# lisqzqng/Video-based-gait-analysis-for-dementia

Hardware: AMD Instinct MI355X
Metric: frames/sec (224x224, seq=16) (higher is better)
Workload: dtype f32

## Files before the change

video-based-gait-analysis-for-dementia_amd/csrc/conv_stem.hip:

```cpp
#include "kernels.h"

namespace grk {

typedef float f32x4 __attribute__((ext_vector_type(4)));

namespace {

__global__ __launch_bounds__(256) void conv_stem_f32(const ConvArgs a) {
    const int lane = threadIdx.x & 63, l15 = lane & 15, lq = lane >> 4;
    const int row = blockIdx.x * 4 + (threadIdx.x >> 6);
    if (row >= a.N * a.Ho) return;
    const int n = row / a.Ho, y = row - n * a.Ho;
    const float* w = a.w;
    float bw[7][4];
#pragma unroll
    for (int s = 0; s < 7; ++s)
#pragma unroll
        for (int nt = 0; nt < 4; ++nt) bw[s][nt] = w[(s * 4 + nt) * 64 + lane];
    float bias[4];
#pragma unroll
    for (int nt = 0; nt < 4; ++nt) bias[nt] = a.bias[nt * 16 + l15];
    const float* rowp[7];
    int kxm1[7];
    bool yok[7];
    const float* inb = a.in + ((size_t)n * a.in_ctot + a.in_coff) * a.H * a.W;
#pragma unroll
    for (int s = 0; s < 7; ++s) {
        const int k = 4 * s + lq, kk = k < 27 ? k : 26, c = kk / 9, t = kk - 9 * c, ky = t / 3, kx = t - 3 * ky;
        const int yin = 2 * y + ky - 1;
        yok[s] = yin >= 0 && yin < a.H;
        rowp[s] = inb + ((size_t)c * a.H + (yok[s] ? yin : 0)) * a.W;
        kxm1[s] = kx - 1;
    }
    auto fetch = [&](int x0, float (&v)[7]) {
#pragma unroll
        for (int s = 0; s < 7; ++s) {
            const int xi = 2 * (x0 + l15) + kxm1[s];
            const bool ok = yok[s] && xi >= 0 && xi < a.W;
            const float t = rowp[s][ok ? xi : 0];
            v[s] = ok ? t : 0.f;
        }
    };
    float cur[7], nxt[7];
    fetch(0, cur);
    float* ob = a.out + (((size_t)n * a.out_ctot + a.out_coff + l15) * a.Ho + y) * a.Wo + 4 * lq;
    const size_t cstride = (size_t)16 * a.Ho * a.Wo;
    for (int x0 = 0; x0 < a.Wo; x0 += 16) {
        fetch(x0 + 16 < a.Wo ? x0 + 16 : x0, nxt);
        f32x4 acc[4];
#pragma unroll
        for (int nt = 0; nt < 4; ++nt) acc[nt] = f32x4{0.f, 0.f, 0.f, 0.f};
#pragma unroll
        for (int s = 0; s < 7; ++s)
#pragma unroll
            for (int nt = 0; nt < 4; ++nt) acc[nt] = __builtin_amdgcn_mfma_f32_16x16x4f32(cur[s], bw[s][nt], acc[nt], 0, 0, 0);
#pragma unroll
        for (int nt = 0; nt < 4; ++nt) {
            f32x4 v = acc[nt] + bias[nt];
            if (a.relu) {
#pragma unroll
                for (int r = 0; r < 4; ++r) v[r] = fmaxf(v[r], 0.f);
            }
            *reinterpret_cast<f32x4*>(ob + nt * cstride + x0) = v;
        }
#pragma unroll
        for (int s = 0; s < 7; ++s) cur[s] = nxt[s];
    }
}

}

bool conv_stem_eligible(int cin, int cout, int ks, int stride, int h, int w, int n_add) {
    return cin == 3 && cout == 64 && ks == 3 && stride == 2 && n_add == 0 && h % 2 == 0 && w % 32 == 0;
}

void pack_stem_weights(const double* w_folded , float* out ) {
    for (int s = 0; s < 7; ++s)
        for (int nt = 0; nt < 4; ++nt)
            for (int lq = 0; lq < 4; ++lq)
                for (int l15 = 0; l15 < 16; ++l15) {
                    const int k = 4 * s + lq, co = 16 * nt + l15;
                    out[(s * 4 + nt) * 64 + lq * 16 + l15] = k < 27 ? (float)w_folded[(size_t)co * 27 + k] : 0.f;
                }
}

hipError_t launch_conv_stem(ConvArgs a, hipStream_t s) {
    if (!conv_stem_eligible(a.Cin, a.Cout, a.ks, a.stride, a.H, a.W, a.n_add) || a.Ho * 2 != a.H || a.Wo * 2 != a.W) return hipErrorInvalidValue;
    const int rows = a.N * a.Ho;
    return launch_k(conv_stem_f32, dim3((rows + 3) / 4), dim3(256), 0, s, a);
}

}
```

video-based-gait-analysis-for-dementia_amd/csrc/grnet.cpp:

```cpp
#include "../../include/grnet_hip.h"

#include <hip/hip_runtime.h>

#include <cmath>
#include <cstdio>
#include <cstdlib>
#include <algorithm>
#include <cstring>
#include <map>
#include <memory>
#include <string>
#include <tuple>
#include <unordered_map>
#include <vector>

#include "kernels.h"

using namespace grk;

namespace grk { thread_local GraphRecorder* g_recorder = nullptr; }

namespace {

constexpr double kBnEps = 1e-5;
// ... 2040 lines not shown
        GraphKey key{n, frames, o};
        auto it = graphs.find(key);
        constexpr size_t kMaxGraphs = 16;
        if (it == graphs.end()) {
            bool seen = false;
            for (const GraphKey& k : seen_once) seen |= !(k < key) && !(key < k);
            if (!seen) {
                if (seen_once.size() >= 64) seen_once.erase(seen_once.begin());
                seen_once.push_back(key);
                return enqueue(frames, n, o, s);
            }
            if (graphs.size() >= kMaxGraphs) {
                auto lru = graphs.begin();
                for (auto g = graphs.begin(); g != graphs.end(); ++g)
                    if (g->second.last_use < lru->second.last_use) lru = g;
                (void)hipGraphExecDestroy(lru->second.exec);
                graphs.erase(lru);
            }
        }
        if (it == graphs.end()) {
            hipGraph_t g = nullptr;
            HIP_TRY(hipGraphCreate(&g, 0));
            GraphRecorder recorder;
            recorder.graph = g;
            static const int edges_env = GRNET_AB(GRAPH_EDGES, 0);
            recorder.edge_order = edges_env;
            g_recorder = &recorder;
            int rc = enqueue(frames, n, o, s);
            g_recorder = nullptr;
            if (rc) { hipGraphDestroy(g); return rc; }
            hipError_t e = hipSuccess;
            if (recorder.edge_order) {
                auto add = [&](std::vector<hipGraphNode_t>& from, std::vector<hipGraphNode_t>& to) {
                    if (e == hipSuccess && !from.empty()) e = hipGraphAddDependencies(g, from.data(), to.data(), from.size());
                };
                if (recorder.edge_order == 2) { add(recorder.cross_from, recorder.cross_to); add(recorder.chain_from, recorder.chain_to); }
                else { add(recorder.chain_from, recorder.chain_to); add(recorder.cross_from, recorder.cross_to); }
                if (e != hipSuccess) { hipGraphDestroy(g); return fail(GRNET_EHIP, std::string("hipGraphAddDependencies: ") + hipGetErrorString(e)); }
            }
            hipGraphExec_t ge = nullptr;
            e = hipGraphInstantiate(&ge, g, nullptr, nullptr, 0);
            hipGraphDestroy(g);
            if (e != hipSuccess) return fail(GRNET_EHIP, std::string("hipGraphInstantiate: ") + hipGetErrorString(e));
            it = graphs.emplace(key, GraphEntry{ge, 0}).first;
        }
        it->second.last_use = ++graph_clock;
        HIP_TRY(hipGraphLaunch(it->second.exec, s));
        return 0;
    }
};

extern "C" {

const char* grnet_version(void) { return "grnet_hip 0.1 (gfx950, fp32 MFMA)"; }

int grnet_create(grnet_t** out_handle, int device_id, int dtype, int max_frames) {
    if (!out_handle || max_frames < 1 || max_frames > 2048 || (dtype != 0 && dtype != 1)) return GRNET_EINVAL;
    *out_handle = nullptr;
    int ndev = 0;
    if (hipGetDeviceCount(&ndev) != hipSuccess || device_id < 0 || device_id >= ndev) return GRNET_EHIP;
    DeviceGuard guard(device_id);
    std::unique_ptr<grnet> h(new grnet());
    h->device = device_id;
    h->max_frames = max_frames;
    h->dtype = dtype;
    if (const char* ml = getenv("GRNET_MULTI_LANE")) h->multi_lane = atoi(ml) != 0;
    if (const char* wn = getenv("GRNET_WINO")) h->wino_mode = atoi(wn) != 0;
    h->build_plan();
    int rc = h->allocate();
    if (rc) { fprintf(stderr, "grnet_create: %s\n", h->err.c_str()); return rc; }
    if (conv_init() != hipSuccess || conv_bf16_init() != hipSuccess || conv_bf16_chain_init() != hipSuccess || conv_bf16_roll_init() != hipSuccess) { fprintf(stderr, "grnet_create: conv_init failed\n"); return GRNET_EHIP; }
    *out_handle = h.release();
    return 0;
}

int grnet_load_tensor(grnet_t* h, const char* key, const void* host_ptr, const int64_t* shape, int ndim, int dtype) {
    if (!h || !key || (!host_ptr && ndim >= 0 && dtype == GRNET_DTYPE_F32) || ndim < 0 || ndim > 8) return GRNET_EINVAL;
    if (h->finalized) return h->fail(GRNET_ESTATE, "grnet_load_tensor after grnet_finalize_weights");
    if (dtype == GRNET_DTYPE_I64) return 0;
    if (dtype != GRNET_DTYPE_F32) return h->fail(GRNET_EINVAL, std::string("unsupported dtype for ") + key);
    HostTensor t;
    size_t numel = 1;
    for (int i = 0; i < ndim; ++i) { t.shape.push_back(shape[i]); numel *= (size_t)shape[i]; }
    t.data.assign(static_cast<const float*>(host_ptr), static_cast<const float*>(host_ptr) + numel);
    h->tensors[key] = std::move(t);
    return 0;
}

int grnet_load_smpl(grnet_t* h, const float* v_template, const float* shapedirs, const float* posedirs, const float* J_regressor,
                    const float* lbs_weights, const int32_t* parents, const float* J_regressor_extra) {
    if (!h || !v_template || !shapedirs || !posedirs || !J_regressor || !lbs_weights || !parents || !J_regressor_extra)
        return GRNET_EINVAL;
    DeviceGuard guard(h->device);
    const int V = 6890;
    for (int i = 0; i < 24; ++i)
        if (parents[i] >= i || (i > 0 && parents[i] < 0)) return h->fail(GRNET_EINVAL, "SMPL parents must be topologically ordered");
    auto up = [&](const float* src, size_t n, const float** dst) {
        std::vector<float> tmp(src, src + n);
        float* p = nullptr;
        int rc = h->upload(tmp, &p);
        *dst = p;
        return rc;
    };
    int rc;
    {
        const size_t C = (size_t)V * 3;
        std::vector<float> blend((size_t)kBlendK * C, 0.f);
// ... 680 lines not shown
```

video-based-gait-analysis-for-dementia_amd/csrc/head_kernels.hip:

```cpp
#include "kernels.h"

namespace grk {

#define GRK_TRY(expr) do { hipError_t _e = (expr); if (_e != hipSuccess) return _e; } while (0)

typedef float f32x4 __attribute__((ext_vector_type(4)));
typedef float f32x2 __attribute__((ext_vector_type(2)));

__device__ __forceinline__ float wave_sum(float v) {
#pragma unroll
    for (int o = 32; o > 0; o >>= 1) v += __shfl_xor(v, o, 64);
    return v;
}
__device__ __forceinline__ float wave_max(float v) {
#pragma unroll
    for (int o = 32; o > 0; o >>= 1) v = fmaxf(v, __shfl_xor(v, o, 64));
    return v;
}

__global__ __launch_bounds__(256) void fuse_sum_kernel(const SumArgs a) {
    const int HW = a.H * a.W, n = blockIdx.x / a.C, c = blockIdx.x - n * a.C;
    const float inv_w = 1.0f / (float)a.W;
    for (int pix = threadIdx.x * 4; pix < HW; pix += 1024) {
        f32x4 v = f32x4{0.f, 0.f, 0.f, 0.f};
// ... 174 lines not shown
    double m[6];
#pragma unroll
    for (int k = 0; k < 6; ++k) m[k] = maps[(size_t)n * mstride + k];
    const int iw = mstride >= 10 ? (int)maps[(size_t)n * mstride + 6] : 0, ih = mstride >= 10 ? (int)maps[(size_t)n * mstride + 7] : 0;
    const double t2[6] = {1.0, 0.0, iw > 0 ? maps[(size_t)n * mstride + 8] : 0.0, 0.0, 1.0, iw > 0 ? maps[(size_t)n * mstride + 9] : 0.0};
    const float mean[3] = {0.485f, 0.456f, 0.406f}, stdv[3] = {0.229f, 0.224f, 0.225f};
    for (int i = blockIdx.x * 256 + threadIdx.x; i < 224 * 224; i += gridDim.x * 256) {
        const int y = i / 224, x = i - y * 224;
        int val[3];
        if (iw <= 0) {
            cv_warp_px(src, H, W, m, x, y, val);
        } else {
            const int X0 = cv_round((t2[1] * y + t2[2]) * 1024.0) + 16, Y0 = cv_round((t2[4] * y + t2[5]) * 1024.0) + 16;
            const int X = (X0 + cv_round(t2[0] * x * 1024.0)) >> 5, Y = (Y0 + cv_round(t2[3] * x * 1024.0)) >> 5;
            const int sx = min(max(X >> 5, -32768), 32767), sy = min(max(Y >> 5, -32768), 32767);
            const int ax = X & 31, ay = Y & 31;
            const int wt[4] = {(32 - ax) * (32 - ay), ax * (32 - ay), (32 - ax) * ay, ax * ay};
            int sum[3] = {0, 0, 0};
#pragma unroll
            for (int t = 0; t < 4; ++t) {
                const int ix = sx + (t & 1), iy = sy + (t >> 1);
                if (wt[t] != 0 && ix >= 0 && ix < iw && iy >= 0 && iy < ih) {
                    int v[3];
                    cv_warp_px(src, H, W, m, ix, iy, v);
                    sum[0] += v[0] * wt[t]; sum[1] += v[1] * wt[t]; sum[2] += v[2] * wt[t];
                }
            }
#pragma unroll
            for (int c = 0; c < 3; ++c) val[c] = (sum[c] * 32 + 16384) >> 15;
        }
#pragma unroll
        for (int c = 0; c < 3; ++c) out[((size_t)n * 3 + c) * (224 * 224) + i] = ((float)val[bgr ? 2 - c : c] / 255.f - mean[c]) / stdv[c];
    }
}

hipError_t launch_crop_normalise_cv(const unsigned char* img, int H, int W, int per_image, const double* maps, int mstride, int bgr, float* out, int N,
                                    hipStream_t s) {
    if (mstride != 6 && mstride != 10) return hipErrorInvalidValue;
    GRK_TRY(launch_k(crop_normalise_cv_kernel, dim3(49, N), dim3(256), 0, s, img, H, W, per_image, maps, mstride, bgr, out));
    return hipSuccess;
}

hipError_t launch_crop_normalise(const unsigned char* img, int H, int W, int per_image, const float* bbox, float scale, int bgr,
                                 float* out, int N, hipStream_t s) {
    GRK_TRY(launch_k(crop_normalise_kernel, dim3(49, N), dim3(256), 0, s, img, H, W, per_image, bbox, scale, bgr, out));
    return hipSuccess;
}

constexpr int kPoolChunk = 448, kPoolStride = kPoolChunk + 4;
__global__ __launch_bounds__(384) void attn_pool_kernel(const float* __restrict__ heat, int heat_ctot, float* __restrict__ stats,
                                                          const float* __restrict__ featA, int CA, const float* __restrict__ featB,
                                                          int CB, float* __restrict__ part, int P) {
    __shared__ __align__(16) float prob[32 * kPoolStride];
    const int n = blockIdx.x, tid = threadIdx.x, lane = tid & 63, l15 = lane & 15, lq = lane >> 4;
    const int pbeg = blockIdx.z * kPoolChunk;
    for (int u = tid; u < 32 * (kPoolChunk / 4); u += 384) {
        const int j = u / (kPoolChunk / 4), q = u - j * (kPoolChunk / 4);
        f32x4 v = {0.f, 0.f, 0.f, 0.f};
        if (j < 24) v = *reinterpret_cast<const f32x4*>(heat + ((size_t)n * heat_ctot + 1 + j) * P + pbeg + 4 * q);
        *reinterpret_cast<f32x4*>(prob + j * kPoolStride + 4 * q) = v;
    }
    __syncthreads();
    for (int j = (tid >> 6) * 4; j < (tid >> 6) * 4 + 4; ++j) {
        float* row = prob + j * kPoolStride;
        float hv[kPoolChunk / 64], m = -INFINITY;
#pragma unroll
        for (int i = 0; i < kPoolChunk / 64; ++i) { hv[i] = row[lane + 64 * i]; m = fmaxf(m, hv[i]); }
        m = wave_max(m);
        float sum = 0.f;
#pragma unroll
        for (int i = 0; i < kPoolChunk / 64; ++i) { const float e = expf(hv[i] - m); row[lane + 64 * i] = e; sum += e; }
        sum = wave_sum(sum);
        if (lane == 0 && blockIdx.y == 0) {
            float* st = stats + (((size_t)n * kPoolSplit + blockIdx.z) * 24 + j) * 2;
            st[0] = m;
            st[1] = sum;
        }
    }
    const int ct = blockIdx.y * 6 + (tid >> 6);
    const int c = ct * 16 + l15;
    const float* frow = (c < CA ? featA + ((size_t)n * CA + c) * P : featB + ((size_t)n * CB + (c - CA)) * P) + pbeg + 4 * lq;
    f32x4 fa[4];
#pragma unroll
    for (int g = 0; g < 4; ++g) fa[g] = *reinterpret_cast<const f32x4*>(frow + 16 * g);
    __syncthreads();
    const float* b0 = prob + l15 * kPoolStride + 4 * lq;
    const float* b1 = prob + (16 + l15) * kPoolStride + 4 * lq;
    f32x4 acc0 = {0.f, 0.f, 0.f, 0.f}, acc1 = {0.f, 0.f, 0.f, 0.f};
    for (int p0 = 0; p0 < kPoolChunk; p0 += 64) {
        const int pn = p0 + 64 < kPoolChunk ? p0 + 64 : p0;
#pragma unroll
        for (int g = 0; g < 4; ++g) {
            const f32x4 f = fa[g];
            fa[g] = *reinterpret_cast<const f32x4*>(frow + pn + 16 * g);
            const f32x4 u = *reinterpret_cast<const f32x4*>(b0 + p0 + 16 * g), v = *reinterpret_cast<const f32x4*>(b1 + p0 + 16 * g);
#pragma unroll
            for (int k = 0; k < 4; ++k) {
                acc0 = __builtin_amdgcn_mfma_f32_16x16x4f32(f[k], u[k], acc0, 0, 0, 0);
                acc1 = __builtin_amdgcn_mfma_f32_16x16x4f32(f[k], v[k], acc1, 0, 0, 0);
            }
        }
    }
    float* o = part + (((size_t)n * kPoolSplit + blockIdx.z) * (CA + CB) + ct * 16 + 4 * lq) * 24;
#pragma unroll
    for (int r = 0; r < 4; ++r) {
        o[r * 24 + l15] = acc0[r];
        if (l15 < 8) o[r * 24 + 16 + l15] = acc1[r];
    }
}

size_t softmax_pool_ws_floats(int N) { return (size_t)N * kPoolStatsFloats + (size_t)N * kPoolSplit * 192 * 24; }

hipError_t launch_softmax_pool(const float* heat, int heat_ctot, const float* featA, int CA, const float* featB, int CB,
                               float* outA, float* outB, float* stats_ws, int N, int P, hipStream_t s) {
    (void)outA; (void)outB;
    if (CA != 128 || CB != 64 || P != kPoolChunk * kPoolSplit) return hipErrorInvalidValue;
    float* part = stats_ws + (size_t)N * kPoolStatsFloats;
    GRK_TRY(launch_k(attn_pool_kernel, dim3(N, (CA + CB) / 96, kPoolSplit), dim3(384), 0, s, heat, heat_ctot, stats_ws, featA, CA, featB,
                       CB, part, P));
    return hipGetLastError();
}

__device__ __forceinline__ void rot6d_to_rotmat_dev(const float* x, float* R) {
    const float a1x = x[0], a1y = x[2], a1z = x[4], a2x = x[1], a2y = x[3], a2z = x[5];
    const float n1 = fmaxf(sqrtf(a1x * a1x + a1y * a1y + a1z * a1z), 1e-6f);
    const float b1x = a1x / n1, b1y = a1y / n1, b1z = a1z / n1;
    const float d = b1x * a2x + b1y * a2y + b1z * a2z;
    const float ux = a2x - d * b1x, uy = a2y - d * b1y, uz = a2z - d * b1z;
    const float n2 = fmaxf(sqrtf(ux * ux + uy * uy + uz * uz), 1e-6f);
    const float b2x = ux / n2, b2y = uy / n2, b2z = uz / n2;
    const float b3x = b1y * b2z - b1z * b2y, b3y = b1z * b2x - b1x * b2z, b3z = b1x * b2y - b1y * b2x;
    R[0] = b1x; R[1] = b2x; R[2] = b3x;
    R[3] = b1y; R[4] = b2y; R[5] = b3y;
    R[6] = b1z; R[7] = b2z; R[8] = b3z;
}

__device__ __forceinline__ void rotmat_to_aa_dev(const float* R, float* aa) {
    const float m00 = R[0], m01 = R[3], m02 = R[6];
    const float m10 = R[1], m11 = R[4], m12 = R[7];
    const float m20 = R[2], m21 = R[5], m22 = R[8];
    float q0, q1, q2, q3, t;
    if (m22 < 1e-6f) {
        if (m00 > m11) { t = 1.f + m00 - m11 - m22; q0 = m12 - m21; q1 = t; q2 = m01 + m10; q3 = m20 + m02; }
        else           { t = 1.f - m00 + m11 - m22; q0 = m20 - m02; q1 = m01 + m10; q2 = t; q3 = m12 + m21; }
    } else {
        if (m00 < -m11) { t = 1.f - m00 - m11 + m22; q0 = m01 - m10; q1 = m20 + m02; q2 = m12 + m21; q3 = t; }
        else            { t = 1.f + m00 + m11 + m22; q0 = t; q1 = m12 - m21; q2 = m20 - m02; q3 = m01 - m10; }
    }
    const float sc = 0.5f / sqrtf(t);
    q0 *= sc; q1 *= sc; q2 *= sc; q3 *= sc;
    const float s2 = q1 * q1 + q2 * q2 + q3 * q3;
    const float sn = sqrtf(s2);
    const float two_theta = 2.f * (q0 < 0.f ? atan2f(-sn, -q0) : atan2f(sn, q0));
    const float k = s2 > 0.f ? two_theta / sn : 2.f;
    float a0 = q1 * k, a1 = q2 * k, a2 = q3 * k;
    aa[0] = isnan(a0) ? 0.f : a0;
    aa[1] = isnan(a1) ? 0.f : a1;
    aa[2] = isnan(a2) ? 0.f : a2;
}

template <bool FROM_PARTS>
__global__ __launch_bounds__(256) void head_tail_kernel(const float* __restrict__ part, const float* __restrict__ zstats, float* __restrict__ plf, float* __restrict__ csf, TailWeights w,
                                                          float* __restrict__ rot6d, float* __restrict__ shape,
                                                          float* __restrict__ cam, float* __restrict__ rotmat,
                                                          float* __restrict__ theta) {
    __shared__ float s_plf[128 * 24];
    __shared__ __align__(16) float s_csf[64 * 24];
    __shared__ float s_pose[24 * 6];
    __shared__ float s_sc[13];
    __shared__ float s_pp[4][144];
// ... 351 lines not shown
```

video-based-gait-analysis-for-dementia_amd/csrc/hr_fuse.hip:

```cpp
#include "kernels.h"

namespace grk {

typedef float f32x4 __attribute__((ext_vector_type(4)));
typedef float f32x2 __attribute__((ext_vector_type(2)));

namespace {

template <int LW> struct VecOf;
template <> struct VecOf<1> { typedef float type; };
template <> struct VecOf<2> { typedef f32x2 type; };
template <> struct VecOf<4> { typedef f32x4 type; };
__device__ __forceinline__ float comp(float v, int) { return v; }
__device__ __forceinline__ float comp(f32x2 v, int r) { return v[r]; }
__device__ __forceinline__ float comp(f32x4 v, int r) { return v[r]; }

template <int NB, int I>
struct OutGeom {
    static constexpr int CI = 32 << I, WI = 56 >> I, BR = 8 >> I, NSRC = NB - 1 - I, NT = CI / 16;
    static constexpr int NSPLIT = NT < 4 ? NT : 4, KS = 4 / NSPLIT, NPW = NT / NSPLIT;
    static constexpr int VW = WI % 4 == 0 ? 4 : 2, WV = WI / VW, NV = CI * BR * WV;
};
template <int NB, int I, int S>
struct SrcGeom {
// ... 29 lines not shown
    }
#pragma unroll
    for (int g = 0; g < Q::KSW / 4; ++g)
#pragma unroll
        for (int u = 0; u < G::NPW; ++u)
            R.b[g][u] = *reinterpret_cast<const f32x4*>(src.w + ((size_t)((ksel * (Q::KSW / 4) + g) * G::NT + nsel * G::NPW + u) * 64 + lane) * 4);
}

template <int NB, int I, int S>
__device__ __forceinline__ void src_compute(const SrcRegs<NB, I, S>& R, float* T, int lane, int nsel, int ksel) {
    typedef SrcGeom<NB, I, S> Q;
    typedef OutGeom<NB, I> G;
    const int l15 = lane & 15, lq = lane >> 4;
    f32x4 acc[Q::MT][G::NPW];
#pragma unroll
    for (int t = 0; t < Q::MT; ++t)
#pragma unroll
        for (int u = 0; u < G::NPW; ++u) acc[t][u] = f32x4{0.f, 0.f, 0.f, 0.f};
#pragma unroll
    for (int ks = 0; ks < Q::KSW; ++ks)
#pragma unroll
        for (int q = 0; q < Q::NLOAD; ++q)
#pragma unroll
            for (int r = 0; r < Q::LW; ++r)
#pragma unroll
                for (int u = 0; u < G::NPW; ++u)
                    acc[q * Q::LW + r][u] = __builtin_amdgcn_mfma_f32_16x16x4f32(comp(R.a[ks][q], r), R.b[ks >> 2][u][ks & 3], acc[q * Q::LW + r][u], 0, 0, 0);
    float* Ts = T + ksel * (TOff<NB, I, G::NSRC>::v) + TOff<NB, I, S>::v;
#pragma unroll
    for (int q = 0; q < Q::NLOAD; ++q)
#pragma unroll
        for (int r = 0; r < Q::LW; ++r)
#pragma unroll
            for (int u = 0; u < G::NPW; ++u) {
                const int c = (nsel * G::NPW + u) * 16 + l15;
#pragma unroll
                for (int e = 0; e < 4; ++e) {
                    const int pix = q * 16 * Q::LW + (4 * lq + e) * Q::LW + r;
                    if (pix < Q::PJ) Ts[c * Q::PJP + pix] = acc[q * Q::LW + r][u][e];
                }
            }
}

template <int NB, int I, int S>
__device__ __forceinline__ float src_term(const float* T, int c, int yl, int x) {
    typedef SrcGeom<NB, I, S> Q;
    typedef OutGeom<NB, I> G;
    const float* Ts = T + TOff<NB, I, S>::v + c * Q::PJP + (yl >> Q::SH) * Q::WJ + (x >> Q::SH);
    float v = Ts[0];
    if constexpr (G::KS == 2) v += Ts[TOff<NB, I, G::NSRC>::v];
    return v;
}

template <int NB, int I>
__device__ __forceinline__ void fuse_up_body(const FuseUpOut& o, int n, int band, float* T) {
    typedef OutGeom<NB, I> G;
    static_assert(G::NSRC >= 1 && G::NSRC <= 3 && G::NV % 256 == 0, "geometry");
    const int tid = threadIdx.x, lane = tid & 63, wave = __builtin_amdgcn_readfirstlane(tid >> 6);
    const int nsel = wave % G::NSPLIT, ksel = wave / G::NSPLIT;
    {
        SrcRegs<NB, I, 0> r0;
        src_load<NB, I, 0>(r0, o.src[0], n, band, lane, nsel, ksel);
        if constexpr (G::NSRC == 1) {
            src_compute<NB, I, 0>(r0, T, lane, nsel, ksel);
        } else {
            SrcRegs<NB, I, 1> r1;
            src_load<NB, I, 1>(r1, o.src[1], n, band, lane, nsel, ksel);
            if constexpr (G::NSRC == 2) {
                src_compute<NB, I, 0>(r0, T, lane, nsel, ksel);
                src_compute<NB, I, 1>(r1, T, lane, nsel, ksel);
            } else {
                SrcRegs<NB, I, 2> r2;
                src_load<NB, I, 2>(r2, o.src[2], n, band, lane, nsel, ksel);
                src_compute<NB, I, 0>(r0, T, lane, nsel, ksel);
                src_compute<NB, I, 1>(r1, T, lane, nsel, ksel);
                src_compute<NB, I, 2>(r2, T, lane, nsel, ksel);
            }
        }
    }
    typedef typename VecOf<G::VW>::type vec;
    vec basev[G::NV / 256];
    float biasv[G::NV / 256];
    const size_t plane = (size_t)G::WI * G::WI;
#pragma unroll
    for (int it = 0; it < G::NV / 256; ++it) {
        const int e = it * 256 + tid, c = e / (G::BR * G::WV), rem = e - c * (G::BR * G::WV), yl = rem / G::WV, xv = rem - yl * G::WV;
        const int pos = (band * G::BR + yl) * G::WI + xv * G::VW;
        basev[it] = *reinterpret_cast<const vec*>(o.base + ((size_t)n * o.base_ctot + o.base_coff + c) * plane + pos);
        if constexpr (I >= 1) {
            if (o.n_extra >= 1) basev[it] += *reinterpret_cast<const vec*>(o.extra[0] + ((size_t)n * o.extra_ctot[0] + o.extra_coff[0] + c) * plane + pos);
            if constexpr (I >= 2) { if (o.n_extra >= 2) basev[it] += *reinterpret_cast<const vec*>(o.extra[1] + ((size_t)n * o.extra_ctot[1] + o.extra_coff[1] + c) * plane + pos); }
        }
        biasv[it] = o.bias[c];
    }
    __syncthreads();
#pragma unroll
    for (int it = 0; it < G::NV / 256; ++it) {
        const int e = it * 256 + tid, c = e / (G::BR * G::WV), rem = e - c * (G::BR * G::WV), yl = rem / G::WV, xv = rem - yl * G::WV;
        vec y = basev[it];
#pragma unroll
        for (int r = 0; r < G::VW; ++r) {
            const int x = xv * G::VW + r;
            float v = y[r] + biasv[it];
            v += src_term<NB, I, 0>(T, c, yl, x);
            if constexpr (G::NSRC >= 2) v += src_term<NB, I, 1>(T, c, yl, x);
            if constexpr (G::NSRC >= 3) v += src_term<NB, I, 2>(T, c, yl, x);
            y[r] = o.relu ? fmaxf(v, 0.f) : v;
        }
        *reinterpret_cast<vec*>(o.out + ((size_t)n * o.out_ctot + o.out_coff + c) * plane + (band * G::BR + yl) * G::WI + xv * G::VW) = y;
    }
}

template <int NB, int I> constexpr int lds_floats() { return OutGeom<NB, I>::KS * TOff<NB, I, OutGeom<NB, I>::NSRC>::v; }
template <int NB> constexpr int lds_floats_max() {
    int m = lds_floats<NB, 0>();
    if constexpr (NB >= 3) m = lds_floats<NB, 1>() > m ? lds_floats<NB, 1>() : m;
    if constexpr (NB >= 4) m = lds_floats<NB, 2>() > m ? lds_floats<NB, 2>() : m;
    return m;
}

template <int NB>
__global__ __launch_bounds__(256) void hr_fuse_up_f32(const FuseUpArgs a) {
    __shared__ __align__(16) float T[lds_floats_max<NB>()];
    const int per = a.N * 7, i = blockIdx.x / per, rem = blockIdx.x - i * per, n = rem / 7, band = rem - n * 7;
    if (i == 0) fuse_up_body<NB, 0>(a.o[0], n, band, T);
    if constexpr (NB >= 3) { if (i == 1) fuse_up_body<NB, 1>(a.o[1], n, band, T); }
    if constexpr (NB >= 4) { if (i == 2) fuse_up_body<NB, 2>(a.o[2], n, band, T); }
}

}

void pack_fuse_up_weights(const double* w, int cout, int cin, float* out) {
    const int nt_n = cout / 16;
    for (int g = 0; g < cin / 16; ++g)
        for (int nt = 0; nt < nt_n; ++nt)
            for (int l = 0; l < 64; ++l)
                for (int kk = 0; kk < 4; ++kk)
                    out[(((size_t)g * nt_n + nt) * 64 + l) * 4 + kk] = (float)w[(size_t)(nt * 16 + (l & 15)) * cin + 16 * g + 4 * kk + (l >> 4)];
}

hipError_t launch_hr_fuse_up(const FuseUpArgs& a, hipStream_t s) {
    if (a.N < 1 || a.nb < 2 || a.nb > 4) return hipErrorInvalidValue;
    const dim3 grid(a.N * 7 * (a.nb - 1));
    if (a.nb == 2) return launch_k(hr_fuse_up_f32<2>, grid, dim3(256), 0, s, a);
    if (a.nb == 3) return launch_k(hr_fuse_up_f32<3>, grid, dim3(256), 0, s, a);
    return launch_k(hr_fuse_up_f32<4>, grid, dim3(256), 0, s, a);
}


namespace {

typedef __bf16 bf16x8_f __attribute__((ext_vector_type(8)));
typedef unsigned int u32x4_f __attribute__((ext_vector_type(4)));
typedef unsigned int u32x2_f __attribute__((ext_vector_type(2)));
typedef unsigned short u16_f;
typedef __bf16 bf16x2_f __attribute__((ext_vector_type(2)));
__device__ __forceinline__ unsigned pack2_f(float lo, float hi) { return __builtin_bit_cast(unsigned, __builtin_convertvector(f32x2{lo, hi}, bf16x2_f)); }
__device__ __forceinline__ void add8_f(float (&acc)[8], u32x4_f v) {
#pragma unroll
    for (int k = 0; k < 4; ++k) { acc[2 * k] += __uint_as_float(v[k] << 16); acc[2 * k + 1] += __uint_as_float(v[k] & 0xffff0000u); }
}

template <int NB, int I>
struct OutGeomB {
    static constexpr int CI = 32 << I, WI = 56 >> I, BR = 8 >> I, NSRC = NB - 1 - I, NCB = CI / 16, UPP = CI / 8;
    static constexpr int NU = BR * WI * UPP, NIT = (NU + 255) / 256;
};
template <int NB, int I, int S>
struct SrcGeomB {
    typedef OutGeomB<NB, I> G;
    static constexpr int J = I + 1 + S, CJ = 32 << J, SH = S + 1, WJ = G::WI >> SH, ROWS = G::BR >> SH, PJ = ROWS * WJ, NPT = (PJ + 15) / 16, NK = CJ / 32;
    static constexpr int TILES = NPT * G::NCB;
    static_assert(ROWS >= 1, "band geometry");
};
template <int NB, int I, int S> struct TOffB { static constexpr int v = TOffB<NB, I, S - 1>::v + SrcGeomB<NB, I, S - 1>::PJ * OutGeomB<NB, I>::CI; };
template <int NB, int I> struct TOffB<NB, I, 0> { static constexpr int v = 0; };

template <int NB, int I, int S>
__device__ __forceinline__ void src_tiles_bf16(const FuseUpSrc& src, int n, int band, int lane, int first, u16_f* T) {
    typedef SrcGeomB<NB, I, S> Q;
    typedef OutGeomB<NB, I> G;
    const int l15 = lane & 15, lq = lane >> 4;
    const u16_f* xb = reinterpret_cast<const u16_f*>(src.x) + (size_t)n * Q::WJ * Q::WJ * src.ctot + src.coff + (size_t)band * Q::PJ * src.ctot;
    const u16_f* wb = reinterpret_cast<const u16_f*>(src.w);
    u16_f* Ts = T + TOffB<NB, I, S>::v;
#pragma unroll
    for (int t = 0; t < (Q::TILES + 3) / 4; ++t) {
        const int tile = first + 4 * t;
        if (tile >= Q::TILES) break;
        const int pt = tile / G::NCB, cb = tile - pt * G::NCB, px = pt * 16 + l15;
        const u16_f* xp = xb + (size_t)(px < Q::PJ ? px : 0) * src.ctot + lq * 8;
        const u16_f* wp = wb + ((size_t)cb * 16 + l15) * 32 + lq * 8;
        bf16x8_f bq[Q::NK], aq[Q::NK];
#pragma unroll
        for (int k = 0; k < Q::NK; ++k) {
            bq[k] = *reinterpret_cast<const bf16x8_f*>(xp + k * 32);
// ... 116 lines not shown
```

video-based-gait-analysis-for-dementia_amd/csrc/kernels.h:

```cpp
#pragma once
#include <hip/hip_runtime.h>
#include <stdint.h>

#include <mutex>
#include <tuple>
#include <utility>
#include <vector>

#ifdef GRNET_ABLATION
#include <cstdlib>
#define GRNET_AB(name, dflt) (getenv("GRNET_" #name) ? atoi(getenv("GRNET_" #name)) : (dflt))
#define GRNET_AB_F(name, dflt) (getenv("GRNET_" #name) ? atof(getenv("GRNET_" #name)) : (dflt))
#define GRNET_AB_SET(name) (getenv("GRNET_" #name) != nullptr)
#define GRNET_AB_STR(name) getenv("GRNET_" #name)
#else
#define GRNET_AB(name, dflt) (dflt)
#define GRNET_AB_F(name, dflt) (dflt)
#define GRNET_AB_SET(name) false
#define GRNET_AB_STR(name) (static_cast<const char*>(nullptr))
#endif

namespace grk {

struct PerDeviceOnce {
// ... 100 lines not shown
    const float* in2; int in2_ctot, in2_coff, cin_split;
    int R, G, Rin, Wp, PSTR, tiles_y, groups, TC, rows;
    float inv_RW, inv_Wo, inv_upc;
    int nbuf;
    int gx, gy, gx8, xcd;
    int pw_stream;
    int dbg;
    int prio;
    int blk0, wsplit;
};

hipError_t launch_conv(ConvArgs a, hipStream_t s, int tile_hint = 0);
struct ConvChoice { int family = 0, tps = 0, tcs = 0, nw = 0, waves = 0, width_variant = 0, rows = 0; };
hipError_t conv_choose(const ConvArgs& a, int tile_hint, ConvChoice* out);
int conv_pick_tc(int Cout);
hipError_t conv_init();
const char* conv_dominant_kernel_name();

bool conv_wino4_eligible(int cin, int cout, int ks, int stride, int h, int w, int n_add);
hipError_t launch_conv_wino4(ConvArgs a, hipStream_t s, int* n_launches = nullptr);
void pack_wino4_weights(const double* w_folded , int cout, int cin, int cin_pad, int cout_pad, float* out, int map_width = 56);
int conv_wino4_blocks(int cout, int map_width);
int conv_wino4_wide(int cout, int map_width);
struct Wino4Form { int waves = 0, nb = 0, npw = 0, gx = 0, gy = 0, xcd = 0, split = 0, full = 0, rest = 0; };
hipError_t conv_wino4_form(const ConvArgs& a, Wino4Form* f);

void wino4_transform_filter(const double* g33, double* u36);
bool conv_pw_eligible(int cin, int cout, int ks, int stride, int h, int w, int n_add);
hipError_t launch_conv_pw(ConvArgs a, hipStream_t s);
bool conv_stem_eligible(int cin, int cout, int ks, int stride, int h, int w, int n_add);
hipError_t launch_conv_stem(ConvArgs a, hipStream_t s);
void pack_stem_weights(const double* w_folded , float* out );
bool conv_wino4s_eligible(int cin, int cout, int ks, int stride, int h, int w, int n_add);
hipError_t launch_conv_wino4s(ConvArgs a, hipStream_t s, int ksplit);
int conv_wino4s_images_per_tile(int map_width);
int conv_wino4s_row_tiles(int map_width, int n_images, int* last_tile_images);
void pack_wino4r_weights(const double* w_folded , int cout, int cin, float* out );
struct SumArgs {
    float* out; int out_ctot, out_coff;
    int N, C, H, W, relu, n_add;
    const float* add[4]; int add_ctot[4], add_coff[4], add_shift[4];
};
hipError_t launch_fuse_sum(const SumArgs& a, hipStream_t s);

struct FuseUpSrc { const float* x; int ctot, coff; const float* w; };
struct FuseUpOut {
    float* out; int out_ctot, out_coff;
    const float* base; int base_ctot, base_coff;
    const float* bias;
    int relu, n_extra;
    const float* extra[2]; int extra_ctot[2], extra_coff[2];
    FuseUpSrc src[3];
};
struct FuseUpArgs { int N, nb; FuseUpOut o[3]; int only = -1; };
hipError_t launch_hr_fuse_up(const FuseUpArgs& a, hipStream_t s);
void pack_fuse_up_weights(const double* w_folded , int cout, int cin, float* out );
hipError_t launch_hr_fuse_up_bf16(const FuseUpArgs& a, hipStream_t s);
void pack_fuse_up_weights_bf16(const double* w_folded , int cout, int cin, unsigned short* out );

hipError_t launch_bilinear2x(const float* in, float* out, int N, int C, int H, int W, hipStream_t s);

hipError_t launch_crop_normalise(const unsigned char* img, int H, int W, int per_image, const float* bbox, float scale, int bgr,
                                 float* out, int N, hipStream_t s);

hipError_t launch_crop_normalise_cv(const unsigned char* img, int H, int W, int per_image, const double* maps, int mstride, int bgr, float* out, int N,
                                    hipStream_t s);

hipError_t launch_softmax_pool(const float* heat, int heat_ctot, const float* featA, int CA, const float* featB, int CB,
                               float* outA, float* outB, float* prob_ws, int N, int P, hipStream_t s);

struct TailWeights {
    const float* pose_w;
    const float* shape_w;
    const float* shape_b;
    const float* cam_w;
    const float* cam_b;
};
hipError_t launch_head_tail(const float* pool_ws, bool range_stats , float* plf, float* csf, TailWeights w, float* rot6d, float* shape, float* cam,
                            float* rotmat, float* theta, int N, hipStream_t s);
hipError_t launch_head_tail_from_feats(const float* plf, const float* csf, TailWeights w, float* rot6d, float* shape, float* cam, float* rotmat,
                                       float* theta, int N, hipStream_t s);
hipError_t launch_rot6d_to_rotmat(const float* x, float* R, int m, hipStream_t s);
hipError_t launch_rotmat_to_aa(const float* R, float* aa, int m, hipStream_t s);
size_t softmax_pool_ws_floats(int N);
constexpr int kPoolStatsFloats = 7 * 24 * 2;
constexpr int kPoolSplit = 7;

constexpr int kBlendK = 220;
constexpr int kSmplWsFloatsPerFrame = 288 + kBlendK;
struct SmplTables {
    const float* blend;
    const int* skin_idx;
    const float* skin_w;
    int skin_k;
    const float* J_template;
    const float* J_shapedirs;
    const float* lbs_weights;
    const int* thorax_idx;
    const float* thorax_w;
    int thorax_n;
    const int* parents;
};
hipError_t launch_smpl(const float* betas, const float* rotmat, const float* cam, SmplTables t, float* A_ws,
                       float* verts, float* kp3d, float* kp2d, int N, hipStream_t s);

constexpr int kJregMaxRows = 64;
constexpr int kJregSlices = 27;
// ... 90 lines not shown
```

Baseline: 4547.

## Prefetch loads earlier in stem conv, attention pool and HR fuse kernels

The stem convolution now gathers inputs for seven column tiles before running their MFMAs, instead of double-buffering one tile. Its bias and ReLU handling becomes branch-free, and out-of-range taps read a zero weight slot. The attention-pool kernel issues its heat-map and feature loads into registers before the softmax, and the NB=2 HR fuse kernel loads base and bias before the compute phase. Block indices in the fuse kernel are also remapped so that work is grouped per XCD. Each change tries to hide global memory latency behind compute, at the cost of more register pressure and lower occupancy. The old variants are kept behind ablation flags.

After: 4541. About the same (-0.1%).

```diff
diff --git a/video-based-gait-analysis-for-dementia_amd/csrc/conv_stem.hip b/video-based-gait-analysis-for-dementia_amd/csrc/conv_stem.hip
--- a/video-based-gait-analysis-for-dementia_amd/csrc/conv_stem.hip
+++ b/video-based-gait-analysis-for-dementia_amd/csrc/conv_stem.hip
@@ -6,7 +6,73 @@
 
 namespace {
 
+constexpr int kStemAhead = 7;
 __global__ __launch_bounds__(256) void conv_stem_f32(const ConvArgs a) {
+    const int lane = threadIdx.x & 63, l15 = lane & 15, lq = lane >> 4;
+    const int row = blockIdx.x * 4 + (threadIdx.x >> 6);
+    if (row >= a.N * a.Ho) return;
+    const int n = row / a.Ho, y = row - n * a.Ho;
+    const float* rowp[7];
+    int kxm1[7];
+    bool yok[7];
+    const float* inb = a.in + ((size_t)n * a.in_ctot + a.in_coff) * a.H * a.W;
+#pragma unroll
+    for (int s = 0; s < 7; ++s) {
+        const int k = 4 * s + lq, kk = k < 27 ? k : 26, c = kk / 9, t = kk - 9 * c, ky = t / 3, kx = t - 3 * ky;
+        const int yin = 2 * y + ky - 1;
+        yok[s] = yin >= 0 && yin < a.H;
+        rowp[s] = inb + ((size_t)c * a.H + (yok[s] ? yin : 0)) * a.W;
+        kxm1[s] = kx - 1;
+    }
+    float* ob = a.out + (((size_t)n * a.out_ctot + a.out_coff + l15) * a.Ho + y) * a.Wo + 4 * lq;
+    const size_t cstride = (size_t)16 * a.Ho * a.Wo;
+    const float* w = a.w;
+    const float* zero = w + (6 * 4) * 64 + 3 * 16;
+    const float floor = a.relu ? 0.f : -INFINITY;
+    for (int xc = 0; xc < a.Wo; xc += 16 * kStemAhead) {
+        float v[kStemAhead][7];
+#pragma unroll
+        for (int t = 0; t < kStemAhead; ++t) {
+            const int x0 = xc + 16 * t < a.Wo ? xc + 16 * t : a.Wo - 16;
+#pragma unroll
+            for (int s = 0; s < 7; ++s) {
+                const int xi = 2 * (x0 + l15) + kxm1[s];
+                const bool ok = yok[s] && xi >= 0 && xi < a.W;
+                v[t][s] = *(ok ? rowp[s] + xi : zero);
+            }
+        }
+        float bw[7][4], bias[4];
+#pragma unroll
+        for (int s = 0; s < 7; ++s)
+#pragma unroll
+            for (int nt = 0; nt < 4; ++nt) bw[s][nt] = w[(s * 4 + nt) * 64 + lane];
+#pragma unroll
+        for (int nt = 0; nt < 4; ++nt) bias[nt] = a.bias[nt * 16 + l15];
+        __builtin_amdgcn_sched_barrier(0);
+#pragma unroll
+        for (int t = 0; t < kStemAhead; ++t) {
+            const int x0 = xc + 16 * t;
+            if (x0 >= a.Wo) break;
+            f32x4 acc[4];
+#pragma unroll
+            for (int nt = 0; nt < 4; ++nt) acc[nt] = f32x4{0.f, 0.f, 0.f, 0.f};
+#pragma unroll
+            for (int s = 0; s < 7; ++s)
+#pragma unroll
+                for (int nt = 0; nt < 4; ++nt) acc[nt] = __builtin_amdgcn_mfma_f32_16x16x4f32(v[t][s], bw[s][nt], acc[nt], 0, 0, 0);
+#pragma unroll
+            for (int nt = 0; nt < 4; ++nt) {
+                f32x4 o = acc[nt] + bias[nt];
+#pragma unroll
+                for (int r = 0; r < 4; ++r) o[r] = fmaxf(o[r], floor);
+                *reinterpret_cast<f32x4*>(ob + nt * cstride + x0) = o;
+            }
+        }
+    }
+}
+
+#ifdef GRNET_ABLATION
+__global__ __launch_bounds__(256) void conv_stem_f32_v0(const ConvArgs a) {
     const int lane = threadIdx.x & 63, l15 = lane & 15, lq = lane >> 4;
     const int row = blockIdx.x * 4 + (threadIdx.x >> 6);
     if (row >= a.N * a.Ho) return;
@@ -67,6 +133,7 @@
         for (int s = 0; s < 7; ++s) cur[s] = nxt[s];
     }
 }
+#endif
 
 }
 
@@ -87,6 +154,9 @@
 hipError_t launch_conv_stem(ConvArgs a, hipStream_t s) {
     if (!conv_stem_eligible(a.Cin, a.Cout, a.ks, a.stride, a.H, a.W, a.n_add) || a.Ho * 2 != a.H || a.Wo * 2 != a.W) return hipErrorInvalidValue;
     const int rows = a.N * a.Ho;
+#ifdef GRNET_ABLATION
+    if (!GRNET_AB(STEM_AHEAD, 1)) return launch_k(conv_stem_f32_v0, dim3((rows + 3) / 4), dim3(256), 0, s, a);
+#endif
     return launch_k(conv_stem_f32, dim3((rows + 3) / 4), dim3(256), 0, s, a);
 }
 
diff --git a/video-based-gait-analysis-for-dementia_amd/csrc/grnet.cpp b/video-based-gait-analysis-for-dementia_amd/csrc/grnet.cpp
--- a/video-based-gait-analysis-for-dementia_amd/csrc/grnet.cpp
+++ b/video-based-gait-analysis-for-dementia_amd/csrc/grnet.cpp
@@ -2116,7 +2116,11 @@
 
 extern "C" {
 
+#ifdef GRNET_ABLATION
+const char* grnet_version(void) { return "grnet_hip 0.1 (gfx950, fp32 MFMA), diagnostic build"; }
+#else
 const char* grnet_version(void) { return "grnet_hip 0.1 (gfx950, fp32 MFMA)"; }
+#endif
 
 int grnet_create(grnet_t** out_handle, int device_id, int dtype, int max_frames) {
     if (!out_handle || max_frames < 1 || max_frames > 2048 || (dtype != 0 && dtype != 1)) return GRNET_EINVAL;
diff --git a/video-based-gait-analysis-for-dementia_amd/csrc/head_kernels.hip b/video-based-gait-analysis-for-dementia_amd/csrc/head_kernels.hip
--- a/video-based-gait-analysis-for-dementia_amd/csrc/head_kernels.hip
+++ b/video-based-gait-analysis-for-dementia_amd/csrc/head_kernels.hip
@@ -250,6 +250,75 @@
                                                           const float* __restrict__ featA, int CA, const float* __restrict__ featB,
                                                           int CB, float* __restrict__ part, int P) {
     __shared__ __align__(16) float prob[32 * kPoolStride];
+    constexpr int kQ = kPoolChunk / 4, kHeatIt = 24 * kQ / 384, kGroups = kPoolChunk / 16;
+    static_assert(24 * kQ % 384 == 0, "the 24 heat-map rows are whole rounds of the workgroup");
+    const int n = blockIdx.x, tid = threadIdx.x, lane = tid & 63, l15 = lane & 15, lq = lane >> 4;
+    const int pbeg = blockIdx.z * kPoolChunk;
+    f32x4 hv4[kHeatIt];
+#pragma unroll
+    for (int i = 0; i < kHeatIt; ++i) {
+        const int u = tid + 384 * i, j = u / kQ, q = u - j * kQ;
+        hv4[i] = *reinterpret_cast<const f32x4*>(heat + ((size_t)n * heat_ctot + 1 + j) * P + pbeg + 4 * q);
+    }
+    const int ct = blockIdx.y * 6 + (tid >> 6);
+    const int c = ct * 16 + l15;
+    const float* frow = (c < CA ? featA + ((size_t)n * CA + c) * P : featB + ((size_t)n * CB + (c - CA)) * P) + pbeg + 4 * lq;
+    f32x4 fa[kGroups];
+#pragma unroll
+    for (int g = 0; g < kGroups; ++g) fa[g] = *reinterpret_cast<const f32x4*>(frow + 16 * g);
+#pragma unroll
+    for (int i = 0; i < kHeatIt; ++i) {
+        const int u = tid + 384 * i, j = u / kQ, q = u - j * kQ;
+        *reinterpret_cast<f32x4*>(prob + j * kPoolStride + 4 * q) = hv4[i];
+    }
+    for (int u = tid; u < 8 * kQ; u += 384) {
+        const int j = 24 + u / kQ, q = u % kQ;
+        *reinterpret_cast<f32x4*>(prob + j * kPoolStride + 4 * q) = f32x4{0.f, 0.f, 0.f, 0.f};
+    }
+    __syncthreads();
+    for (int j = (tid >> 6) * 4; j < (tid >> 6) * 4 + 4; ++j) {
+        float* row = prob + j * kPoolStride;
+        float hv[kPoolChunk / 64], m = -INFINITY;
+#pragma unroll
+        for (int i = 0; i < kPoolChunk / 64; ++i) { hv[i] = row[lane + 64 * i]; m = fmaxf(m, hv[i]); }
+        m = wave_max(m);
+        float sum = 0.f;
+#pragma unroll
+        for (int i = 0; i < kPoolChunk / 64; ++i) { const float e = expf(hv[i] - m); row[lane + 64 * i] = e; sum += e; }
+        sum = wave_sum(sum);
+        if (lane == 0 && blockIdx.y == 0) {
+            float* st = stats + (((size_t)n * kPoolSplit + blockIdx.z) * 24 + j) * 2;
+            st[0] = m;
+            st[1] = sum;
+        }
+    }
+    __syncthreads();
+    const float* b0 = prob + l15 * kPoolStride + 4 * lq;
+    const float* b1 = prob + (16 + l15) * kPoolStride + 4 * lq;
+    f32x4 acc0 = {0.f, 0.f, 0.f, 0.f}, acc1 = {0.f, 0.f, 0.f, 0.f};
+#pragma unroll
+    for (int g = 0; g < kGroups; ++g) {
+        const f32x4 f = fa[g];
+        const f32x4 u = *reinterpret_cast<const f32x4*>(b0 + 16 * g), v = *reinterpret_cast<const f32x4*>(b1 + 16 * g);
+#pragma unroll
+        for (int k = 0; k < 4; ++k) {
+            acc0 = __builtin_amdgcn_mfma_f32_16x16x4f32(f[k], u[k], acc0, 0, 0, 0);
+            acc1 = __builtin_amdgcn_mfma_f32_16x16x4f32(f[k], v[k], acc1, 0, 0, 0);
+        }
+    }
+    float* o = part + (((size_t)n * kPoolSplit + blockIdx.z) * (CA + CB) + ct * 16 + 4 * lq) * 24;
+#pragma unroll
+    for (int r = 0; r < 4; ++r) {
+        o[r * 24 + l15] = acc0[r];
+        if (l15 < 8) o[r * 24 + 16 + l15] = acc1[r];
+    }
+}
+
+#ifdef GRNET_ABLATION
+__global__ __launch_bounds__(384) void attn_pool_v0_kernel(const float* __restrict__ heat, int heat_ctot, float* __restrict__ stats,
+                                                          const float* __restrict__ featA, int CA, const float* __restrict__ featB,
+                                                          int CB, float* __restrict__ part, int P) {
+    __shared__ __align__(16) float prob[32 * kPoolStride];
     const int n = blockIdx.x, tid = threadIdx.x, lane = tid & 63, l15 = lane & 15, lq = lane >> 4;
     const int pbeg = blockIdx.z * kPoolChunk;
     for (int u = tid; u < 32 * (kPoolChunk / 4); u += 384) {
@@ -306,6 +375,7 @@
         if (l15 < 8) o[r * 24 + 16 + l15] = acc1[r];
     }
 }
+#endif
 
 size_t softmax_pool_ws_floats(int N) { return (size_t)N * kPoolStatsFloats + (size_t)N * kPoolSplit * 192 * 24; }
 
@@ -314,6 +384,12 @@
     (void)outA; (void)outB;
     if (CA != 128 || CB != 64 || P != kPoolChunk * kPoolSplit) return hipErrorInvalidValue;
     float* part = stats_ws + (size_t)N * kPoolStatsFloats;
+#ifdef GRNET_ABLATION
+    if (!GRNET_AB(POOL_AHEAD, 1)) {
+        GRK_TRY(launch_k(attn_pool_v0_kernel, dim3(N, (CA + CB) / 96, kPoolSplit), dim3(384), 0, s, heat, heat_ctot, stats_ws, featA, CA, featB, CB, part, P));
+        return hipGetLastError();
+    }
+#endif
     GRK_TRY(launch_k(attn_pool_kernel, dim3(N, (CA + CB) / 96, kPoolSplit), dim3(384), 0, s, heat, heat_ctot, stats_ws, featA, CA, featB,
                        CB, part, P));
     return hipGetLastError();
diff --git a/video-based-gait-analysis-for-dementia_amd/csrc/hr_fuse.hip b/video-based-gait-analysis-for-dementia_amd/csrc/hr_fuse.hip
--- a/video-based-gait-analysis-for-dementia_amd/csrc/hr_fuse.hip
+++ b/video-based-gait-analysis-for-dementia_amd/csrc/hr_fuse.hip
@@ -105,47 +105,53 @@
     return v;
 }
 
-template <int NB, int I>
+template <int NB, int I, bool EARLY>
 __device__ __forceinline__ void fuse_up_body(const FuseUpOut& o, int n, int band, float* T) {
     typedef OutGeom<NB, I> G;
     static_assert(G::NSRC >= 1 && G::NSRC <= 3 && G::NV % 256 == 0, "geometry");
     const int tid = threadIdx.x, lane = tid & 63, wave = __builtin_amdgcn_readfirstlane(tid >> 6);
     const int nsel = wave % G::NSPLIT, ksel = wave / G::NSPLIT;
+    typedef typename VecOf<G::VW>::type vec;
+    vec basev[G::NV / 256];
+    float biasv[G::NV / 256];
+    const size_t plane = (size_t)G::WI * G::WI;
+    auto load_base = [&]() {
+#pragma unroll
+        for (int it = 0; it < G::NV / 256; ++it) {
+            const int e = it * 256 + tid, c = e / (G::BR * G::WV), rem = e - c * (G::BR * G::WV), yl = rem / G::WV, xv = rem - yl * G::WV;
+            const int pos = (band * G::BR + yl) * G::WI + xv * G::VW;
+            basev[it] = *reinterpret_cast<const vec*>(o.base + ((size_t)n * o.base_ctot + o.base_coff + c) * plane + pos);
+            if constexpr (I >= 1) {
+                if (o.n_extra >= 1) basev[it] += *reinterpret_cast<const vec*>(o.extra[0] + ((size_t)n * o.extra_ctot[0] + o.extra_coff[0] + c) * plane + pos);
+                if constexpr (I >= 2) { if (o.n_extra >= 2) basev[it] += *reinterpret_cast<const vec*>(o.extra[1] + ((size_t)n * o.extra_ctot[1] + o.extra_coff[1] + c) * plane + pos); }
+            }
+            biasv[it] = o.bias[c];
+        }
+    };
     {
         SrcRegs<NB, I, 0> r0;
         src_load<NB, I, 0>(r0, o.src[0], n, band, lane, nsel, ksel);
         if constexpr (G::NSRC == 1) {
+            if constexpr (EARLY) load_base();
             src_compute<NB, I, 0>(r0, T, lane, nsel, ksel);
         } else {
             SrcRegs<NB, I, 1> r1;
             src_load<NB, I, 1>(r1, o.src[1], n, band, lane, nsel, ksel);
             if constexpr (G::NSRC == 2) {
+                if constexpr (EARLY) load_base();
                 src_compute<NB, I, 0>(r0, T, lane, nsel, ksel);
                 src_compute<NB, I, 1>(r1, T, lane, nsel, ksel);
             } else {
                 SrcRegs<NB, I, 2> r2;
                 src_load<NB, I, 2>(r2, o.src[2], n, band, lane, nsel, ksel);
+                if constexpr (EARLY) load_base();
                 src_compute<NB, I, 0>(r0, T, lane, nsel, ksel);
                 src_compute<NB, I, 1>(r1, T, lane, nsel, ksel);
                 src_compute<NB, I, 2>(r2, T, lane, nsel, ksel);
             }
         }
     }
-    typedef typename VecOf<G::VW>::type vec;
-    vec basev[G::NV / 256];
-    float biasv[G::NV / 256];
-    const size_t plane = (size_t)G::WI * G::WI;
-#pragma unroll
-    for (int it = 0; it < G::NV / 256; ++it) {
-        const int e = it * 256 + tid, c = e / (G::BR * G::WV), rem = e - c * (G::BR * G::WV), yl = rem / G::WV, xv = rem - yl * G::WV;
-        const int pos = (band * G::BR + yl) * G::WI + xv * G::VW;
-        basev[it] = *reinterpret_cast<const vec*>(o.base + ((size_t)n * o.base_ctot + o.base_coff + c) * plane + pos);
-        if constexpr (I >= 1) {
-            if (o.n_extra >= 1) basev[it] += *reinterpret_cast<const vec*>(o.extra[0] + ((size_t)n * o.extra_ctot[0] + o.extra_coff[0] + c) * plane + pos);
-            if constexpr (I >= 2) { if (o.n_extra >= 2) basev[it] += *reinterpret_cast<const vec*>(o.extra[1] + ((size_t)n * o.extra_ctot[1] + o.extra_coff[1] + c) * plane + pos); }
-        }
-        biasv[it] = o.bias[c];
-    }
+    if constexpr (!EARLY) load_base();
     __syncthreads();
 #pragma unroll
     for (int it = 0; it < G::NV / 256; ++it) {
@@ -172,14 +178,37 @@
     return m;
 }
 
+template <int NB, bool EARLY>
+__device__ __forceinline__ void fuse_up_block(const FuseUpArgs& a, float* T) {
+    int b = blockIdx.x, i, n, band;
+    if (a.xcd) {
+        const int x = b & 7, q = gridDim.x >> 3, r = gridDim.x & 7;
+        b = x * q + (x < r ? x : r) + (b >> 3);
+        n = b / (7 * (NB - 1));
+        const int k = b - n * (7 * (NB - 1));
+        i = k / 7, band = k - i * 7;
+    } else {
+        const int per = a.N * 7, rem = b % per;
+        i = b / per, n = rem / 7, band = rem - n * 7;
+    }
+    if (i == 0) fuse_up_body<NB, 0, EARLY>(a.o[0], n, band, T);
+    if constexpr (NB >= 3) { if (i == 1) fuse_up_body<NB, 1, EARLY>(a.o[1], n, band, T); }
+    if constexpr (NB >= 4) { if (i == 2) fuse_up_body<NB, 2, EARLY>(a.o[2], n, band, T); }
+}
+
 template <int NB>
 __global__ __launch_bounds__(256) void hr_fuse_up_f32(const FuseUpArgs a) {
     __shared__ __align__(16) float T[lds_floats_max<NB>()];
-    const int per = a.N * 7, i = blockIdx.x / per, rem = blockIdx.x - i * per, n = rem / 7, band = rem - n * 7;
-    if (i == 0) fuse_up_body<NB, 0>(a.o[0], n, band, T);
-    if constexpr (NB >= 3) { if (i == 1) fuse_up_body<NB, 1>(a.o[1], n, band, T); }
-    if constexpr (NB >= 4) { if (i == 2) fuse_up_body<NB, 2>(a.o[2], n, band, T); }
-}
+    fuse_up_block<NB, NB == 2>(a, T);
+}
+
+#ifdef GRNET_ABLATION
+template <int NB>
+__global__ __launch_bounds__(256) void hr_fuse_up_f32_v0(const FuseUpArgs a) {
+    __shared__ __align__(16) float T[lds_floats_max<NB>()];
+    fuse_up_block<NB, false>(a, T);
+}
+#endif
 
 }
 
@@ -192,9 +221,18 @@
                     out[(((size_t)g * nt_n + nt) * 64 + l) * 4 + kk] = (float)w[(size_t)(nt * 16 + (l & 15)) * cin + 16 * g + 4 * kk + (l >> 4)];
 }
 
-hipError_t launch_hr_fuse_up(const FuseUpArgs& a, hipStream_t s) {
-    if (a.N < 1 || a.nb < 2 || a.nb > 4) return hipErrorInvalidValue;
+hipError_t launch_hr_fuse_up(const FuseUpArgs& a_in, hipStream_t s) {
+    if (a_in.N < 1 || a_in.nb < 2 || a_in.nb > 4) return hipErrorInvalidValue;
+    FuseUpArgs a = a_in;
+    a.xcd = GRNET_AB(FUSE_XCD, 1);
     const dim3 grid(a.N * 7 * (a.nb - 1));
+#ifdef GRNET_ABLATION
+    if (!GRNET_AB(FUSE_EARLY, 1)) {
+        if (a.nb == 2) return launch_k(hr_fuse_up_f32_v0<2>, grid, dim3(256), 0, s, a);
+        if (a.nb == 3) return launch_k(hr_fuse_up_f32_v0<3>, grid, dim3(256), 0, s, a);
+        return launch_k(hr_fuse_up_f32_v0<4>, grid, dim3(256), 0, s, a);
+    }
+#endif
     if (a.nb == 2) return launch_k(hr_fuse_up_f32<2>, grid, dim3(256), 0, s, a);
     if (a.nb == 3) return launch_k(hr_fuse_up_f32<3>, grid, dim3(256), 0, s, a);
     return launch_k(hr_fuse_up_f32<4>, grid, dim3(256), 0, s, a);
diff --git a/video-based-gait-analysis-for-dementia_amd/csrc/kernels.h b/video-based-gait-analysis-for-dementia_amd/csrc/kernels.h
--- a/video-based-gait-analysis-for-dementia_amd/csrc/kernels.h
+++ b/video-based-gait-analysis-for-dementia_amd/csrc/kernels.h
@@ -176,7 +176,7 @@
     const float* extra[2]; int extra_ctot[2], extra_coff[2];
     FuseUpSrc src[3];
 };
-struct FuseUpArgs { int N, nb; FuseUpOut o[3]; int only = -1; };
+struct FuseUpArgs { int N, nb; FuseUpOut o[3]; int only = -1; int xcd = 0; };
 hipError_t launch_hr_fuse_up(const FuseUpArgs& a, hipStream_t s);
 void pack_fuse_up_weights(const double* w_folded , int cout, int cin, float* out );
 hipError_t launch_hr_fuse_up_bf16(const FuseUpArgs& a, hipStream_t s);
```
